# papuSpartan/stable-diffusion-webui-distributed

Measured on AMD Instinct MI355X. Metric: images/sec (whole node) SD1.5 txt2img 512x512 20-step batch=64 at 1/2/4/8 GPU, higher is better.
Workload: dtype bf16; 1 GPU; task=txt2img, model=sd15, global_batch=64, seq_len=512, resolution=512x512, denoise_steps=20, sampler=Euler a, parallelism=dp1 (benchmark-weighted batch shard)

## Files before the change

sdwd_amd/ops/hip/conv.hip:

```cpp
#include "common.h"
#include <map>
#include <mutex>
#include <tuple>

typedef __attribute__((ext_vector_type(4))) float f32x4c;

#define CONV_BM 128
#define CONV_BN 128
#define CONV_BK 64
#define TILE_ELEMS (CONV_BM * CONV_BK)


template <bool HAS_BIAS, bool HAS_RES, bool HAS_CB, int BN = 128,
          bool UPS = false, bool WRAP = false, bool FOLD = false>
__launch_bounds__(256, 2) __global__ void conv3x3_nhwc_bf16_kernel(
    const __hip_bfloat16 *__restrict__ X,
    const __hip_bfloat16 *__restrict__ Wt,
    const float *__restrict__ bias,
    const __hip_bfloat16 *__restrict__ Res,
    const __hip_bfloat16 *__restrict__ CB,
    const __hip_bfloat16 *__restrict__ Zero,
    __hip_bfloat16 *__restrict__ Y,
    int Nn, int H, int W, int Cin, int Cout, int Ho, int Wo, int stride,
    int ldY, float *__restrict__ GNP = nullptr, int wrap_h = 0,
    int wrap_w = 0) {
  __shared__ __align__(16) __bf16 smem[4 * TILE_ELEMS];

  static_assert(!(UPS && FOLD) && !(FOLD && (HAS_RES || HAS_CB)));
  const long M = FOLD ? (long)Nn * H * W : (long)Nn * Ho * Wo;
  constexpr int NJ = BN / 32;
  constexpr int BTILE = BN * CONV_BK;
  const int fa = FOLD ? (blockIdx.y >> 1) & 1 : 0;
  const int fb = FOLD ? blockIdx.y & 1 : 0;
  const long m0 =
      (((long)blockIdx.y + (long)blockIdx.z * 32768) >> (FOLD ? 2 : 0)) *
      CONV_BM;
  if constexpr (FOLD) {
    if (m0 >= M) return;
  }
  const int n0 = blockIdx.x * BN;

  const int tid = threadIdx.x;
  const int lane = tid % WAVE;
  const int wid = tid / WAVE;
  const int wm = (wid >> 1) * 64;
  const int wn = (wid & 1) * (BN / 2);

  long abase[4];
  int hs[4], ws[4];
  int bco[4];
  constexpr int NB = BN / 32;
  int nimg[4];
#pragma unroll
  for (int i = 0; i < 4; ++i) {
    const int row = i * 32 + wid * 8 + lane / 8;
    const long m = m0 + row;
    const long mm = (m < M) ? m : (M - 1);
    if constexpr (FOLD) {
      const unsigned q = (unsigned)mm / (unsigned)W;
      hs[i] = (int)(q % (unsigned)H) - 1 + fa;
      ws[i] = (int)((unsigned)mm - q * (unsigned)W) - 1 + fb;
      nimg[i] = 0;
      abase[i] = (mm + (long)(fa - 1) * W + (fb - 1)) * Cin;
    } else {
      const int n_img = (int)(mm / ((long)Ho * Wo));
      const int rem = (int)(mm % ((long)Ho * Wo));
      hs[i] = (rem / Wo) * stride;
      ws[i] = (rem % Wo) * stride;
      nimg[i] = n_img;
      abase[i] = (((long)n_img * H + hs[i]) * W + ws[i]) * Cin;
    }
    bco[i] = n0 + row;
  }
  const int schunk = lane % 8;

  const int kc_per_plane = Cin / CONV_BK;
  const int NT = (FOLD ? 4 : 9) * kc_per_plane;
  const int row_elems = W * Cin, img_elems = H * row_elems;
  (void)row_elems;
  (void)img_elems;

  auto stage = [&](int t, int b) {
    const int plane = t / kc_per_plane;
    const int kc = t % kc_per_plane;
    const int dy = FOLD ? plane >> 1 : plane / 3 - 1;
    const int dx = FOLD ? plane & 1 : plane % 3 - 1;
    const long poff = ((long)dy * W + dx) * Cin + (long)kc * CONV_BK;
    __bf16 *abuf = smem + b * (TILE_ELEMS + BTILE);
    __bf16 *bbuf = abuf + TILE_ELEMS;
#pragma unroll
    for (int i = 0; i < 4; ++i) {
      const int row = i * 32 + wid * 8 + lane / 8;
      const int sc = cswz(row, schunk);
      bool av;
      const __hip_bfloat16 *asrc;
      if constexpr (WRAP && UPS) {
        int vh = hs[i] + dy, vw = ws[i] + dx;
        if (wrap_h) {
          vh += vh < 0 ? 2 * H : 0;
          vh -= vh >= 2 * H ? 2 * H : 0;
        }
        if (wrap_w) {
          vw += vw < 0 ? 2 * W : 0;
          vw -= vw >= 2 * W ? 2 * W : 0;
        }
        av = vh >= 0 && vh < 2 * H && vw >= 0 && vw < 2 * W;
        asrc = av ? (X +
                     (((long)nimg[i] * H + (vh >> 1)) * W + (vw >> 1)) *
                         Cin +
                     (long)kc * CONV_BK + sc * 8)
                  : Zero;
      } else if constexpr (WRAP) {
        const int hh = hs[i] + dy, ww = ws[i] + dx;
        int dlt = 0;
        if (wrap_h) dlt += hh < 0 ? img_elems : (hh >= H ? -img_elems : 0);
        if (wrap_w) dlt += ww < 0 ? row_elems : (ww >= W ? -row_elems : 0);
        av = (wrap_h || (hh >= 0 && hh < H)) &&
             (wrap_w || (ww >= 0 && ww < W));
        asrc = av ? (X + abase[i] + poff + dlt + sc * 8) : Zero;
      } else if constexpr (UPS) {
        const int vh = hs[i] + dy, vw = ws[i] + dx;
        av = vh >= 0 && vh < 2 * H && vw >= 0 && vw < 2 * W;
        asrc = av ? (X +
                     (((long)nimg[i] * H + (vh >> 1)) * W + (vw >> 1)) *
                         Cin +
                     (long)kc * CONV_BK + sc * 8)
                  : Zero;
      } else {
        av = (hs[i] + dy >= 0) && (hs[i] + dy < H) &&
             (ws[i] + dx >= 0) && (ws[i] + dx < W);
        asrc = av ? (X + abase[i] + poff + sc * 8) : Zero;
      }
      (void)poff;
      __builtin_amdgcn_global_load_lds(
          (const __attribute__((address_space(1))) unsigned int *)asrc,
          (__attribute__((address_space(3))) unsigned int
               *)(abuf + i * 2048 + wid * 512),
          16, 0, 0);
      if (i < NB) {
        const bool bv = bco[i] < Cout;
        const __hip_bfloat16 *bsrc;
        if constexpr (FOLD) {
          bsrc = bv ? (Wt +
                       (((long)(2 * fa + fb) * Cout + bco[i]) * 4 + plane) *
                           Cin +
                       kc * CONV_BK + sc * 8)
                    : Zero;
        } else {
          bsrc = bv ? (Wt + (long)bco[i] * 9 * Cin + plane * Cin +
                       kc * CONV_BK + sc * 8)
                    : Zero;
        }
        __builtin_amdgcn_global_load_lds(
            (const __attribute__((address_space(1))) unsigned int *)bsrc,
            (__attribute__((address_space(3))) unsigned int
                 *)(bbuf + i * 2048 + wid * 512),
            16, 0, 0);
      }
    }
  };

  f32x4c acc[4][NJ];
#pragma unroll
  for (int i = 0; i < 4; ++i)
#pragma unroll
    for (int j = 0; j < NJ; ++j) acc[i][j] = (f32x4c){};

  stage(0, 0);
  if (NT > 1) stage(1, 1);

  const int l16 = lane % 16;
  const int kq = (lane / 16) * 8;

  for (int t = 0; t < NT; ++t) {
    if (t + 1 < NT)
      asm volatile("s_waitcnt vmcnt(%0)" :: "i"(4 + NB) : "memory");
    else
      asm volatile("s_waitcnt vmcnt(0)" ::: "memory");
    __builtin_amdgcn_s_barrier();

    const __bf16 *abuf = smem + (t & 1) * (TILE_ELEMS + BTILE);
    const __bf16 *bbuf = abuf + TILE_ELEMS;
#pragma unroll
    for (int s = 0; s < 2; ++s) {
      bf16x8 af[4], bf[NJ];
#pragma unroll
      for (int i = 0; i < 4; ++i) {
        const int am = wm + i * 16 + l16;
        const int ck = cswz(am, (s * 32 + kq) / 8);
        af[i] = *(const bf16x8 *)((const char *)(abuf + am * CONV_BK) +
                                  ck * 16);
      }
#pragma unroll
      for (int j = 0; j < NJ; ++j) {
        const int bn = wn + j * 16 + l16;
        const int ck = cswz(bn, (s * 32 + kq) / 8);
        bf[j] = *(const bf16x8 *)((const char *)(bbuf + bn * CONV_BK) +
                                  ck * 16);
      }
      __builtin_amdgcn_s_setprio(1);
#pragma unroll
      for (int i = 0; i < 4; ++i)
#pragma unroll
        for (int j = 0; j < NJ; ++j)
          acc[i][j] = __builtin_amdgcn_mfma_f32_16x16x32_bf16(
              af[i], bf[j], acc[i][j], 0, 0, 0);
      __builtin_amdgcn_s_setprio(0);
    }
    __builtin_amdgcn_s_barrier();
    if (t + 2 < NT) stage(t + 2, t & 1);
  }

  const int r4 = (lane / 16) * 4;
  float gs[NJ], gq[NJ];
#pragma unroll
  for (int j = 0; j < NJ; ++j) gs[j] = gq[j] = 0.0f;
#pragma unroll
  for (int i = 0; i < 4; ++i) {
#pragma unroll
    for (int j = 0; j < NJ; ++j) {
      const int co = n0 + wn + j * 16 + l16;
      if (co >= Cout) continue;
      const float bv = HAS_BIAS ? bias[co] : 0.0f;
#pragma unroll
      for (int r = 0; r < 4; ++r) {
        long m = m0 + wm + i * 16 + r4 + r;
        if (m >= M) continue;
        if constexpr (FOLD) {
          const unsigned q = (unsigned)m / (unsigned)W;
          const unsigned jw = (unsigned)m - q * (unsigned)W;
          m = (long)(2 * q + fa) * Wo + 2 * jw + fb;
        }
        float v = acc[i][j][r] + bv;
        if (HAS_CB) {
          const int ni = (int)(m / ((long)Ho * Wo));
          v += (float)CB[(long)ni * ldY + co];
        }
        if (HAS_RES) v += (float)Res[m * ldY + co];
        const __hip_bfloat16 vb = f2bf(v);
        Y[m * ldY + co] = vb;
        if (GNP) {
          const float vr = bf2f(vb);
          gs[j] += vr;
          gq[j] += vr * vr;
        }
      }
    }
  }
  if (GNP) {
    float *lds = (float *)smem;
#pragma unroll
    for (int j = 0; j < NJ; ++j) {
#pragma unroll
      for (int off = 16; off < 64; off <<= 1) {
        gs[j] += __shfl_down(gs[j], off, WAVE);
        gq[j] += __shfl_down(gq[j], off, WAVE);
      }
      if (lane < 16) {
        float *slot = lds + ((wid * NJ + j) * 16 + lane) * 2;
        slot[0] = gs[j];
        slot[1] = gq[j];
      }
    }
    __syncthreads();
    long gslot = (long)blockIdx.y + (long)blockIdx.z * 32768;
    if constexpr (FOLD) {
      const long tps = ((long)H * W) / CONV_BM, tp = gslot >> 2;
      gslot = ((tp / tps) * 4 + (gslot & 3)) * tps + tp % tps;
    }
    for (int c = tid; c < BN; c += 256) {
      const int co = n0 + c;
      if (co >= Cout) continue;
      const int h = c / (BN / 2);
      const int jj = (c % (BN / 2)) / 16;
      const int lc = c % 16;
      const float *s0 = lds + ((h * NJ + jj) * 16 + lc) * 2;
      const float *s1 = lds + (((h + 2) * NJ + jj) * 16 + lc) * 2;
      float *dst = GNP + (gslot * 2) * (long)ldY;
      dst[co] = s0[0] + s1[0];
      dst[ldY + co] = s0[1] + s1[1];
    }
  }
}

#ifdef __HIP_PLATFORM_AMD__
bool conv3x3_supported(long cin) { return cin % 64 == 0 && cin >= 64; }

std::tuple<long, long, bool> conv3x3_plan(long N, long H, long W, long Cin,
                                          long Cout, long stride,
                                          long force) {
  const long Ho = (H + 2 - 3) / stride + 1;
  const long Wo = (W + 2 - 3) / stride + 1;
  const long M = N * Ho * Wo;
  const long mtiles = (M + CONV_BM - 1) / CONV_BM;
  const long mt4 = (M + V4_BM - 1) / V4_BM;
  const bool v4_shape =
      force == 4 ? (Cin % 64 == 0 && Cout >= 256)
                 : (Cin <= 960 && Cout <= 640 && Cout >= 256 &&
                    mt4 * (Cout / 256) >= 256);
  const long nfull = (force == 2 || !v4_shape) ? 0 : Cout / 256;
  const long rem = Cout - nfull * 256;
  const bool bn64 =
      rem > 0 && (rem <= 64 || mtiles * ((rem + 127) / 128) < 512);
  return {nfull, rem, bn64};
}

static const __hip_bfloat16 *zero_page_for(const torch::Tensor &x) {
  static std::mutex mu;
  static std::map<int, torch::Tensor> pages;
  std::lock_guard<std::mutex> lock(mu);
  auto &page = pages[x.get_device()];
  if (!page.defined()) page = torch::zeros({64}, x.options());
  return (const __hip_bfloat16 *)page.data_ptr();
}

template <class F>
static void dispatch_bools(F &&f) {
  f();
}
template <class F, class... Rest>
static void dispatch_bools(F &&f, bool b, Rest... rest) {
  if (b)
    dispatch_bools([&](auto... cs) { f(std::true_type{}, cs...); }, rest...);
  else
    dispatch_bools([&](auto... cs) { f(std::false_type{}, cs...); }, rest...);
}

static dim3 conv_grid(long col_tiles, long mtiles) {
  return dim3((unsigned)col_tiles, (unsigned)std::min<long>(mtiles, 32768),
              (unsigned)((mtiles + 32767) / 32768));
}

struct ConvArgs {
  int N, Cin, H, W, Cout, Ho, Wo;
  long M;
  torch::Tensor y, gnp, bias_f32, cb_bf16;
  const __hip_bfloat16 *x, *w, *res = nullptr, *cb = nullptr, *zero;
  const float *bias = nullptr;
  __hip_bfloat16 *yp;
  float *gnp_ptr = nullptr;

  ConvArgs(const torch::Tensor &xt, const torch::Tensor &w_prep,
           const c10::optional<torch::Tensor> &bias_t,
           const c10::optional<torch::Tensor> &residual,
           const c10::optional<torch::Tensor> &chan_bias, int Ho_, int Wo_,
           bool collect_gn)
      : N(xt.size(0)), Cin(xt.size(1)), H(xt.size(2)), W(xt.size(3)),
        Cout(w_prep.size(0)), Ho(Ho_), Wo(Wo_), M((long)N * Ho_ * Wo_) {
    TORCH_CHECK(xt.is_contiguous(torch::MemoryFormat::ChannelsLast),
                "conv3x3: x must be channels_last");
    TORCH_CHECK(xt.scalar_type() == torch::kBFloat16);
    TORCH_CHECK(conv3x3_supported(Cin), "conv3x3: Cin % 64 != 0");
    y = torch::empty({N, Cout, Ho, Wo},
                     xt.options().memory_format(
                         torch::MemoryFormat::ChannelsLast));
    x = (const __hip_bfloat16 *)xt.data_ptr();
    w = (const __hip_bfloat16 *)w_prep.data_ptr();
    yp = (__hip_bfloat16 *)y.data_ptr();
    zero = zero_page_for(xt);
    if (bias_t.has_value()) {
      bias_f32 = bias_t->to(torch::kFloat).contiguous();
      bias = bias_f32.data_ptr<float>();
    }
    if (residual.has_value()) {
      TORCH_CHECK(
          residual->is_contiguous(torch::MemoryFormat::ChannelsLast));
      res = (const __hip_bfloat16 *)residual->data_ptr();
    }
    if (chan_bias.has_value()) {
      cb_bf16 = chan_bias->to(torch::kBFloat16).contiguous();
      cb = (const __hip_bfloat16 *)cb_bf16.data_ptr();
    }
    if (collect_gn && ((long)Ho * Wo) % 128 == 0) {
      gnp = torch::empty({M / 128, 2, (long)Cout},
                         xt.options().dtype(torch::kFloat));
      gnp_ptr = gnp.data_ptr<float>();
    }
  }

  std::tuple<torch::Tensor, c10::optional<torch::Tensor>> result() const {
    if (gnp.defined()) return {y, gnp};
    return {y, c10::nullopt};
  }
};

std::tuple<torch::Tensor, c10::optional<torch::Tensor>> conv3x3_nhwc(
    torch::Tensor x, torch::Tensor w_prep, c10::optional<torch::Tensor> bias,
    c10::optional<torch::Tensor> residual,
    c10::optional<torch::Tensor> chan_bias, long stride, bool collect_gn,
    long force, bool wrap_h = false, bool wrap_w = false) {
  const int Ho = (x.size(2) + 2 - 3) / stride + 1;
  const int Wo = (x.size(3) + 2 - 3) / stride + 1;
  ConvArgs a(x, w_prep, bias, residual, chan_bias, Ho, Wo, collect_gn);
  auto stream = cur_stream();
  const bool wrap = wrap_h || wrap_w;
  TORCH_CHECK(!wrap || (long)a.H * a.W * a.Cin < (1L << 31),
              "conv3x3: wrapped image too large");
  const auto [nfull, rem, bn64] =
      conv3x3_plan(a.N, a.H, a.W, a.Cin, a.Cout, stride, force);
  if (nfull > 0) {
    const int cols = (int)(nfull * 256);
    dispatch_bools(
        [&, cols](auto B, auto R, auto C, auto WR) {
          hipLaunchKernelGGL(
              (conv3x3_v4_kernel<decltype(B)::value, decltype(R)::value,
                                 decltype(C)::value, decltype(WR)::value>),
              conv_grid(cols / 256, (a.M + V4_BM - 1) / V4_BM), dim3(512), 0,
              stream, a.x, a.w, a.bias, a.res, a.cb, a.zero, a.yp, a.N, a.H,
              a.W, a.Cin, cols, a.Cout, a.Ho, a.Wo, (int)stride, a.gnp_ptr,
              (int)wrap_h, (int)wrap_w);
        },
        a.bias != nullptr, a.res != nullptr, a.cb != nullptr, wrap);
  }
  if (rem > 0) {
    const long co0 = nfull * 256;
    const int cols = (int)rem;
    dispatch_bools(
        [&, co0, cols](auto B, auto R, auto C, auto N64, auto WR) {
          constexpr int BN = decltype(N64)::value ? 64 : 128;
          hipLaunchKernelGGL(
              (conv3x3_nhwc_bf16_kernel<decltype(B)::value,
                                        decltype(R)::value,
                                        decltype(C)::value, BN, false,
                                        decltype(WR)::value>),
              conv_grid((cols + BN - 1) / BN,
                        (a.M + CONV_BM - 1) / CONV_BM),
              dim3(256), 0, stream, a.x, a.w + co0 * 9 * a.Cin,
              a.bias ? a.bias + co0 : nullptr, a.res ? a.res + co0 : nullptr,
              a.cb ? a.cb + co0 : nullptr, a.zero, a.yp + co0, a.N, a.H, a.W,
              a.Cin, cols, a.Ho, a.Wo, (int)stride, a.Cout,
              a.gnp_ptr ? a.gnp_ptr + co0 : nullptr, (int)wrap_h,
              (int)wrap_w);
        },
        a.bias != nullptr, a.res != nullptr, a.cb != nullptr, bn64, wrap);
  }
  return a.result();
}

static torch::Tensor launch_gn_tile_stats(const torch::Tensor &a,
                                          const torch::Tensor *b,
                                          torch::Tensor *out);

std::tuple<torch::Tensor, c10::optional<torch::Tensor>> ups2x_conv3x3(
    torch::Tensor x, torch::Tensor w_prep, c10::optional<torch::Tensor> bias,
    bool collect_gn, bool wrap_h = false, bool wrap_w = false,
    c10::optional<torch::Tensor> w_fold = c10::nullopt, bool fold = true) {
  auto stream = cur_stream();
  if (fold) {
    TORCH_CHECK(w_fold.has_value(),
                "ups2x_conv3x3: fold needs w_fold (fold_ups2x_weight)");
    const long H = x.size(2), W = x.size(3), Cin = x.size(1);
    const long Cout = w_prep.size(0), Mp = x.size(0) * H * W;
    TORCH_CHECK(w_fold->is_cuda() && w_fold->is_contiguous() &&
                    w_fold->scalar_type() == torch::kBFloat16 &&
                    w_fold->dim() == 5 && w_fold->size(0) == 4 &&
                    w_fold->size(1) == Cout && w_fold->size(2) == 2 &&
                    w_fold->size(3) == 2 && w_fold->size(4) == Cin,
                "ups2x_conv3x3: w_fold must be bf16 [4,Cout,2,2,Cin]");
    TORCH_CHECK(Mp < (1L << 31), "ups2x_conv3x3: too many source pixels");
    TORCH_CHECK(!(wrap_h || wrap_w) || H * W * Cin < (1L << 31),
                "ups2x_conv3x3: wrapped image too large");
    const bool epi_gn = collect_gn && (H * W) % CONV_BM == 0;
    ConvArgs a(x, w_prep, bias, c10::nullopt, c10::nullopt, 2 * H, 2 * W,
               epi_gn);
    const __hip_bfloat16 *wf = (const __hip_bfloat16 *)w_fold->data_ptr();
    dispatch_bools(
        [&](auto B, auto WR) {
          hipLaunchKernelGGL(
              (conv3x3_nhwc_bf16_kernel<decltype(B)::value, false, false,
                                        128, false, decltype(WR)::value,
                                        true>),
              conv_grid((a.Cout + CONV_BN - 1) / CONV_BN,
                        4 * ((Mp + CONV_BM - 1) / CONV_BM)),
              dim3(256), 0, stream, a.x, wf, a.bias, a.res, a.cb, a.zero,
              a.yp, a.N, a.H, a.W, a.Cin, a.Cout, a.Ho, a.Wo, 1, a.Cout,
              a.gnp_ptr, (int)wrap_h, (int)wrap_w);
        },
        a.bias != nullptr, wrap_h || wrap_w);
    if (collect_gn && !epi_gn && ((long)a.Ho * a.Wo) % 128 == 0 &&
        a.Cout % 8 == 0)
      a.gnp = launch_gn_tile_stats(a.y, nullptr, nullptr);
    return a.result();
  }
  ConvArgs a(x, w_prep, bias, c10::nullopt, c10::nullopt, 2 * x.size(2),
             2 * x.size(3), collect_gn);
  dispatch_bools(
      [&](auto B, auto WR) {
        hipLaunchKernelGGL(
            (conv3x3_nhwc_bf16_kernel<decltype(B)::value, false, false, 128,
                                      true, decltype(WR)::value>),
            conv_grid((a.Cout + CONV_BN - 1) / CONV_BN,
                      (a.M + CONV_BM - 1) / CONV_BM),
            dim3(256), 0, stream, a.x, a.w, a.bias, a.res, a.cb, a.zero,
            a.yp, a.N, a.H, a.W, a.Cin, a.Cout, a.Ho, a.Wo, 1, a.Cout,
            a.gnp_ptr, (int)wrap_h, (int)wrap_w);
      },
      a.bias != nullptr, wrap_h || wrap_w);
  return a.result();
}
#endif
```

sdwd_amd/ops/hip/conv_v4.hip:

```cpp
#include "common.h"

__device__ __forceinline__ int cswz(int row, int chunk) {
  return chunk ^ ((row >> 1) & 7);
}

#define V4_BM 256
#define V4_BN 256
#define V4_BK 64
#define V4_ATILE (V4_BM * V4_BK)

template <bool HAS_BIAS, bool HAS_RES, bool HAS_CB, bool WRAP = false>
__launch_bounds__(512, 2) __global__ void conv3x3_v4_kernel(
    const __hip_bfloat16 *__restrict__ X,
    const __hip_bfloat16 *__restrict__ Wt,
    const float *__restrict__ bias,
    const __hip_bfloat16 *__restrict__ Res,
    const __hip_bfloat16 *__restrict__ CB,
    const __hip_bfloat16 *__restrict__ Zero,
    __hip_bfloat16 *__restrict__ Y,
    int Nn, int H, int W, int Cin, int Cols, int ldY, int Ho, int Wo,
    int stride, float *__restrict__ GNP = nullptr, int wrap_h = 0,
    int wrap_w = 0) {
  __shared__ __align__(16) __bf16 smem[4 * V4_ATILE];

  const long M = (long)Nn * Ho * Wo;
  const long m0 =
      ((long)blockIdx.y + (long)blockIdx.z * 32768) * V4_BM;
  const int n0 = blockIdx.x * V4_BN;

  const int tid = threadIdx.x;
  const int lane = tid % WAVE;
  const int wid = tid / WAVE;
  const int wm = (wid >> 2) * 128;
  const int wn = (wid & 3) * 64;

  const int prow = tid / 8;
  const int schunk = tid % 8;
  long abase[4];
  int hs[4], ws[4];
  int bco[4];
#pragma unroll
  for (int i = 0; i < 4; ++i) {
    const long m = m0 + prow + 64 * i;
    const long mm = (m < M) ? m : (M - 1);
    const int n_img = (int)(mm / ((long)Ho * Wo));
    const int rem = (int)(mm % ((long)Ho * Wo));
    hs[i] = (rem / Wo) * stride;
    ws[i] = (rem % Wo) * stride;
    abase[i] = (((long)n_img * H + hs[i]) * W + ws[i]) * Cin;
    bco[i] = n0 + prow + 64 * i;
  }

  const int kc_per_plane = Cin / V4_BK;
  const int NT = 9 * kc_per_plane;
  const int row_elems = W * Cin, img_elems = H * row_elems;
  (void)row_elems;
  (void)img_elems;

  auto stage8 = [&](int t, int b) {
    const int plane = t / kc_per_plane;
    const int kc = t % kc_per_plane;
    const int dy = plane / 3 - 1, dx = plane % 3 - 1;
    const long poff = ((long)dy * W + dx) * Cin + (long)kc * V4_BK;
    __bf16 *abuf = smem + b * (2 * V4_ATILE);
    __bf16 *bbuf = abuf + V4_ATILE;
    const int sc = schunk;
    constexpr int PIECES[8] = {4, 5, 6, 7, 0, 1, 2, 3};
#pragma unroll
    for (int k = 0; k < 8; ++k) {
      const int i = PIECES[k];
      if (i < 4) {
        const int row = prow + 64 * i;
        const int swz = cswz(row, sc);
        bool av;
        const __hip_bfloat16 *asrc;
        if constexpr (WRAP) {
          const int hh = hs[i] + dy, ww = ws[i] + dx;
          int dlt = 0;
          if (wrap_h) dlt += hh < 0 ? img_elems : (hh >= H ? -img_elems : 0);
          if (wrap_w) dlt += ww < 0 ? row_elems : (ww >= W ? -row_elems : 0);
          av = (wrap_h || (hh >= 0 && hh < H)) &&
               (wrap_w || (ww >= 0 && ww < W));
          asrc = av ? (X + abase[i] + poff + dlt + swz * 8) : Zero;
        } else {
          av = (hs[i] + dy >= 0) && (hs[i] + dy < H) &&
               (ws[i] + dx >= 0) && (ws[i] + dx < W);
          asrc = av ? (X + abase[i] + poff + swz * 8) : Zero;
        }
        __builtin_amdgcn_global_load_lds(
            (const __attribute__((address_space(1))) unsigned int *)asrc,
            (__attribute__((address_space(3))) unsigned int
                 *)(abuf + (long)i * 4096 + (long)tid * 8),
            16, 0, 0);
      } else {
        const int bi = i - 4;
        const int row = prow + 64 * bi;
        const int swz = cswz(row, sc);
        const bool bv = bco[bi] < Cols;
        const __hip_bfloat16 *bsrc =
            bv ? (Wt + (long)bco[bi] * 9 * Cin + plane * Cin +
                  kc * V4_BK + swz * 8)
               : Zero;
        __builtin_amdgcn_global_load_lds(
            (const __attribute__((address_space(1))) unsigned int *)bsrc,
            (__attribute__((address_space(3))) unsigned int
                 *)(bbuf + (long)bi * 4096 + (long)tid * 8),
            16, 0, 0);
      }
    }
  };

  f32x4 acc[8][4];
#pragma unroll
  for (int i = 0; i < 8; ++i)
#pragma unroll
    for (int j = 0; j < 4; ++j) acc[i][j] = (f32x4){};

  stage8(0, 0);
  asm volatile("s_waitcnt vmcnt(0)" ::: "memory");
  __builtin_amdgcn_s_barrier();

  const int l16 = lane % 16;
  const int kq4 = lane / 16;

  for (int t = 0; t < NT; ++t) {
    const __bf16 *abuf = smem + (t & 1) * (2 * V4_ATILE);
    const __bf16 *bbuf = abuf + V4_ATILE;
#pragma unroll
    for (int ph = 0; ph < 4; ++ph) {
      const int mh = ph >> 1, nh = ph & 1;
      bf16x8 af[4][2], bf[2][2];
#pragma unroll
      for (int s = 0; s < 2; ++s) {
#pragma unroll
        for (int i = 0; i < 4; ++i) {
          const int ar = wm + mh * 64 + i * 16 + l16;
          const int ck = cswz(ar, s * 4 + kq4);
          af[i][s] = *(const bf16x8 *)((const char *)(abuf +
                                                      (long)ar * V4_BK) +
                                       ck * 16);
        }
#pragma unroll
        for (int j = 0; j < 2; ++j) {
          const int br = wn + nh * 32 + j * 16 + l16;
          const int ck = cswz(br, s * 4 + kq4);
          bf[j][s] = *(const bf16x8 *)((const char *)(bbuf +
                                                      (long)br * V4_BK) +
                                       ck * 16);
        }
      }
      if (ph == 0 && t + 1 < NT) stage8(t + 1, (t + 1) & 1);
      __builtin_amdgcn_s_barrier();
      __builtin_amdgcn_s_setprio(1);
#pragma unroll
      for (int s = 0; s < 2; ++s)
#pragma unroll
        for (int i = 0; i < 4; ++i)
#pragma unroll
          for (int j = 0; j < 2; ++j)
            acc[mh * 4 + i][nh * 2 + j] =
                __builtin_amdgcn_mfma_f32_16x16x32_bf16(
                    af[i][s], bf[j][s], acc[mh * 4 + i][nh * 2 + j], 0, 0,
                    0);
      __builtin_amdgcn_s_setprio(0);
      if (ph == 3 && t + 1 < NT)
        asm volatile("s_waitcnt vmcnt(0)" ::: "memory");
      __builtin_amdgcn_s_barrier();
    }
  }

  const int r4 = (lane / 16) * 4;
  float gs[4], gq[4];
#pragma unroll
  for (int j = 0; j < 4; ++j) gs[j] = gq[j] = 0.0f;
#pragma unroll
  for (int i = 0; i < 8; ++i) {
#pragma unroll
    for (int j = 0; j < 4; ++j) {
      const int co = n0 + wn + (j >> 1) * 32 + (j & 1) * 16 + l16;
      if (co >= Cols) continue;
      const float bv = HAS_BIAS ? bias[co] : 0.0f;
#pragma unroll
      for (int r = 0; r < 4; ++r) {
        const long m = m0 + wm + (i >> 2) * 64 + (i & 3) * 16 + r4 + r;
        if (m >= M) continue;
        float v = acc[i][j][r] + bv;
        if (HAS_CB) {
          const int ni = (int)(m / ((long)Ho * Wo));
          v += (float)CB[(long)ni * ldY + co];
        }
        if (HAS_RES) v += (float)Res[m * ldY + co];
        const __hip_bfloat16 vb = f2bf(v);
        Y[m * ldY + co] = vb;
        if (GNP) {
          const float vr = bf2f(vb);
          gs[j] += vr;
          gq[j] += vr * vr;
        }
      }
    }
  }
  if (GNP) {
    float *lds = (float *)smem;
#pragma unroll
    for (int j = 0; j < 4; ++j) {
#pragma unroll
      for (int off = 16; off < 64; off <<= 1) {
        gs[j] += __shfl_down(gs[j], off, WAVE);
        gq[j] += __shfl_down(gq[j], off, WAVE);
      }
      if (lane < 16) {
        float *slot = lds + ((wid * 4 + j) * 16 + lane) * 2;
        slot[0] = gs[j];
        slot[1] = gq[j];
      }
    }
    __syncthreads();
    const long mt128 = m0 / 128;
    for (int c = tid; c < V4_BN; c += 512) {
      const int co = n0 + c;
      if (co >= Cols) continue;
      const int q = c / 64;
      const int o = c % 64;
      const int jj = (o / 32) * 2 + (o % 32) / 16;
      const int lc = c % 16;
      const float *s0 = lds + ((q * 4 + jj) * 16 + lc) * 2;
      const float *s1 = lds + (((q + 4) * 4 + jj) * 16 + lc) * 2;
      float *d0 = GNP + (mt128 * 2) * (long)ldY;
      d0[co] = s0[0];
      d0[ldY + co] = s0[1];
      if ((mt128 + 1) * 128 < M) {
        float *d1 = GNP + ((mt128 + 1) * 2) * (long)ldY;
        d1[co] = s1[0];
        d1[ldY + co] = s1[1];
      }
    }
  }
}
```

Before: 17.25 images/sec.

## Stage conv epilogue through LDS for vectorized 16-byte output stores

Adds a shared epilogue helper that, for full tiles, writes bias/residual/channel-bias-adjusted bf16 results into per-wave LDS strips and then stores them to global memory as 16-byte vectors instead of scattered 2-byte stores. Residual and channel-bias loads are prefetched one row-group ahead, and the channel-bias division is dropped when a tile lies within a single image. Bias can now be passed as bf16 or fp32 without a host-side conversion. The partial-tile path keeps the scalar epilogue, and the GroupNorm scratch area moves in LDS to avoid overlapping the strips.

New measurement: 18.14 images/sec, median of 6. +5.1%, better.

```diff
diff --git a/sdwd_amd/ops/hip/conv.hip b/sdwd_amd/ops/hip/conv.hip
--- a/sdwd_amd/ops/hip/conv.hip
+++ b/sdwd_amd/ops/hip/conv.hip
@@ -1,4 +1,5 @@
 #include "common.h"
+#include "conv_epilogue.h"
 #include <map>
 #include <mutex>
 #include <tuple>
@@ -16,13 +17,13 @@
 __launch_bounds__(256, 2) __global__ void conv3x3_nhwc_bf16_kernel(
     const __hip_bfloat16 *__restrict__ X,
     const __hip_bfloat16 *__restrict__ Wt,
-    const float *__restrict__ bias,
+    const void *__restrict__ bias,
     const __hip_bfloat16 *__restrict__ Res,
     const __hip_bfloat16 *__restrict__ CB,
     const __hip_bfloat16 *__restrict__ Zero,
     __hip_bfloat16 *__restrict__ Y,
     int Nn, int H, int W, int Cin, int Cout, int Ho, int Wo, int stride,
-    int ldY, float *__restrict__ GNP = nullptr, int wrap_h = 0,
+    int ldY, int flags, float *__restrict__ GNP = nullptr, int wrap_h = 0,
     int wrap_w = 0) {
   __shared__ __align__(16) __bf16 smem[4 * TILE_ELEMS];
 
@@ -215,40 +216,81 @@
   float gs[NJ], gq[NJ];
 #pragma unroll
   for (int j = 0; j < NJ; ++j) gs[j] = gq[j] = 0.0f;
-#pragma unroll
-  for (int i = 0; i < 4; ++i) {
+  const bool full =
+      (flags & CONV_F_VEC) && m0 + CONV_BM <= M && n0 + BN <= Cout;
+  if (full) {
+    const int uw = __builtin_amdgcn_readfirstlane(wid);
+    const int uwm = (uw >> 1) * 64, uwn = (uw & 1) * (BN / 2);
+    float bv[NJ], cbv[NJ];
 #pragma unroll
     for (int j = 0; j < NJ; ++j) {
-      const int co = n0 + wn + j * 16 + l16;
-      if (co >= Cout) continue;
-      const float bv = HAS_BIAS ? bias[co] : 0.0f;
-#pragma unroll
-      for (int r = 0; r < 4; ++r) {
-        long m = m0 + wm + i * 16 + r4 + r;
-        if (m >= M) continue;
-        if constexpr (FOLD) {
-          const unsigned q = (unsigned)m / (unsigned)W;
-          const unsigned jw = (unsigned)m - q * (unsigned)W;
-          m = (long)(2 * q + fa) * Wo + 2 * jw + fb;
+      bv[j] = HAS_BIAS ? conv_bias_at(bias, flags, n0 + uwn + j * 16 + l16)
+                       : 0.0f;
+      cbv[j] = 0.0f;
+    }
+    const unsigned HoWo = (unsigned)(Ho * Wo);
+    bool cb_one = true;
+    unsigned rem0 = 0;
+    const __hip_bfloat16 *cbw = nullptr;
+    if constexpr (HAS_CB) {
+      const long ni0 = m0 / (long)HoWo;
+      const unsigned remb = (unsigned)(m0 - ni0 * (long)HoWo);
+      cb_one = remb + CONV_BM <= HoWo;
+      rem0 = remb + uwm;
+      cbw = CB + ni0 * (long)ldY + n0 + uwn;
+#pragma unroll
+      for (int j = 0; j < NJ; ++j) cbv[j] = (float)cbw[j * 16 + l16];
+    }
+    const long mw = m0 + uwm;
+    const __hip_bfloat16 *resw =
+        HAS_RES ? Res + mw * (long)ldY + n0 + uwn : nullptr;
+    __hip_bfloat16 *yw =
+        FOLD ? Y + n0 + uwn : Y + mw * (long)ldY + n0 + uwn;
+    char *wl = (char *)smem + wid * conv_epi_bytes<NJ>;
+    if (cb_one)
+      conv_epi_strip<HAS_RES, HAS_CB, true, FOLD, NJ, false>(
+          acc, bv, cbv, cbw, rem0, HoWo, resw, yw, mw, W, Wo, fa, fb,
+          (unsigned)ldY, wl, lane, gs, gq);
+    else
+      conv_epi_strip<HAS_RES, HAS_CB, false, FOLD, NJ, false>(
+          acc, bv, cbv, cbw, rem0, HoWo, resw, yw, mw, W, Wo, fa, fb,
+          (unsigned)ldY, wl, lane, gs, gq);
+  } else {
+#pragma unroll
+    for (int i = 0; i < 4; ++i) {
+#pragma unroll
+      for (int j = 0; j < NJ; ++j) {
+        const int co = n0 + wn + j * 16 + l16;
+        if (co >= Cout) continue;
+        const float bv = HAS_BIAS ? conv_bias_at(bias, flags, co) : 0.0f;
+#pragma unroll
+        for (int r = 0; r < 4; ++r) {
+          long m = m0 + wm + i * 16 + r4 + r;
+          if (m >= M) continue;
+          if constexpr (FOLD) {
+            const unsigned q = (unsigned)m / (unsigned)W;
+            const unsigned jw = (unsigned)m - q * (unsigned)W;
+            m = (long)(2 * q + fa) * Wo + 2 * jw + fb;
+          }
+          float v = acc[i][j][r] + bv;
+          if (HAS_CB) {
+            const int ni = (int)(m / ((long)Ho * Wo));
+            v += (float)CB[(long)ni * ldY + co];
+          }
+          if (HAS_RES) v += (float)Res[m * ldY + co];
+          const __hip_bfloat16 vb = f2bf(v);
+          Y[m * ldY + co] = vb;
+          if (GNP) {
+            const float vr = bf2f(vb);
+            gs[j] += vr;
+            gq[j] += vr * vr;
+          }
         }
-        float v = acc[i][j][r] + bv;
-        if (HAS_CB) {
-          const int ni = (int)(m / ((long)Ho * Wo));
-          v += (float)CB[(long)ni * ldY + co];
-        }
-        if (HAS_RES) v += (float)Res[m * ldY + co];
-        const __hip_bfloat16 vb = f2bf(v);
-        Y[m * ldY + co] = vb;
-        if (GNP) {
-          const float vr = bf2f(vb);
-          gs[j] += vr;
-          gq[j] += vr * vr;
-        }
       }
     }
   }
   if (GNP) {
-    float *lds = (float *)smem;
+    float *lds = (float *)((char *)smem + 4 * conv_epi_bytes<4>);
 #pragma unroll
     for (int j = 0; j < NJ; ++j) {
 #pragma unroll
@@ -336,9 +378,19 @@
   long M;
   torch::Tensor y, gnp, bias_f32, cb_bf16;
   const __hip_bfloat16 *x, *w, *res = nullptr, *cb = nullptr, *zero;
-  const float *bias = nullptr;
+  const char *bias = nullptr;
+  int bias_esize = 4;
   __hip_bfloat16 *yp;
   float *gnp_ptr = nullptr;
+
+  const void *bias_at(long co0) const {
+    return bias ? bias + co0 * bias_esize : nullptr;
+  }
+  int flags(long co0, long cols) const {
+    const bool vec = cols % 8 == 0 && Cout % 8 == 0 &&
+                     (reinterpret_cast<uintptr_t>(yp + co0) & 15) == 0;
+    return (vec ? CONV_F_VEC : 0) | (bias_esize == 2 ? CONV_F_BIAS_BF16 : 0);
+  }
 
   ConvArgs(const torch::Tensor &xt, const torch::Tensor &w_prep,
            const c10::optional<torch::Tensor> &bias_t,
@@ -358,9 +410,19 @@
     w = (const __hip_bfloat16 *)w_prep.data_ptr();
     yp = (__hip_bfloat16 *)y.data_ptr();
     zero = zero_page_for(xt);
+    TORCH_CHECK(Cout < (1 << 20), "conv3x3: too many output channels");
+    TORCH_CHECK((long)Ho * Wo < (1L << 30), "conv3x3: output image too large");
     if (bias_t.has_value()) {
-      bias_f32 = bias_t->to(torch::kFloat).contiguous();
-      bias = bias_f32.data_ptr<float>();
+      TORCH_CHECK(bias_t->numel() == Cout, "conv3x3: bias must be [Cout]");
+      const auto bt = bias_t->scalar_type();
+      if ((bt == torch::kBFloat16 || bt == torch::kFloat) &&
+          bias_t->is_contiguous()) {
+        bias_f32 = *bias_t;
+        bias_esize = bt == torch::kBFloat16 ? 2 : 4;
+      } else {
+        bias_f32 = bias_t->to(torch::kFloat).contiguous();
+      }
+      bias = (const char *)bias_f32.data_ptr();
     }
     if (residual.has_value()) {
       TORCH_CHECK(
@@ -406,9 +468,9 @@
               (conv3x3_v4_kernel<decltype(B)::value, decltype(R)::value,
                                  decltype(C)::value, decltype(WR)::value>),
               conv_grid(cols / 256, (a.M + V4_BM - 1) / V4_BM), dim3(512), 0,
-              stream, a.x, a.w, a.bias, a.res, a.cb, a.zero, a.yp, a.N, a.H,
-              a.W, a.Cin, cols, a.Cout, a.Ho, a.Wo, (int)stride, a.gnp_ptr,
-              (int)wrap_h, (int)wrap_w);
+              stream, a.x, a.w, a.bias_at(0), a.res, a.cb, a.zero, a.yp, a.N,
+              a.H, a.W, a.Cin, cols, a.Cout, a.Ho, a.Wo, (int)stride,
+              a.flags(0, cols), a.gnp_ptr, (int)wrap_h, (int)wrap_w);
         },
         a.bias != nullptr, a.res != nullptr, a.cb != nullptr, wrap);
   }
@@ -426,11 +488,11 @@
               conv_grid((cols + BN - 1) / BN,
                         (a.M + CONV_BM - 1) / CONV_BM),
               dim3(256), 0, stream, a.x, a.w + co0 * 9 * a.Cin,
-              a.bias ? a.bias + co0 : nullptr, a.res ? a.res + co0 : nullptr,
+              a.bias_at(co0), a.res ? a.res + co0 : nullptr,
               a.cb ? a.cb + co0 : nullptr, a.zero, a.yp + co0, a.N, a.H, a.W,
               a.Cin, cols, a.Ho, a.Wo, (int)stride, a.Cout,
-              a.gnp_ptr ? a.gnp_ptr + co0 : nullptr, (int)wrap_h,
-              (int)wrap_w);
+              a.flags(co0, cols), a.gnp_ptr ? a.gnp_ptr + co0 : nullptr,
+              (int)wrap_h, (int)wrap_w);
         },
         a.bias != nullptr, a.res != nullptr, a.cb != nullptr, bn64, wrap);
   }
@@ -472,9 +534,10 @@
                                         true>),
               conv_grid((a.Cout + CONV_BN - 1) / CONV_BN,
                         4 * ((Mp + CONV_BM - 1) / CONV_BM)),
-              dim3(256), 0, stream, a.x, wf, a.bias, a.res, a.cb, a.zero,
-              a.yp, a.N, a.H, a.W, a.Cin, a.Cout, a.Ho, a.Wo, 1, a.Cout,
-              a.gnp_ptr, (int)wrap_h, (int)wrap_w);
+              dim3(256), 0, stream, a.x, wf, a.bias_at(0), a.res, a.cb,
+              a.zero, a.yp, a.N, a.H, a.W, a.Cin, a.Cout, a.Ho, a.Wo, 1,
+              a.Cout, a.flags(0, a.Cout), a.gnp_ptr, (int)wrap_h,
+              (int)wrap_w);
         },
         a.bias != nullptr, wrap_h || wrap_w);
     if (collect_gn && !epi_gn && ((long)a.Ho * a.Wo) % 128 == 0 &&
@@ -491,9 +554,9 @@
                                       true, decltype(WR)::value>),
             conv_grid((a.Cout + CONV_BN - 1) / CONV_BN,
                       (a.M + CONV_BM - 1) / CONV_BM),
-            dim3(256), 0, stream, a.x, a.w, a.bias, a.res, a.cb, a.zero,
-            a.yp, a.N, a.H, a.W, a.Cin, a.Cout, a.Ho, a.Wo, 1, a.Cout,
-            a.gnp_ptr, (int)wrap_h, (int)wrap_w);
+            dim3(256), 0, stream, a.x, a.w, a.bias_at(0), a.res, a.cb,
+            a.zero, a.yp, a.N, a.H, a.W, a.Cin, a.Cout, a.Ho, a.Wo, 1,
+            a.Cout, a.flags(0, a.Cout), a.gnp_ptr, (int)wrap_h, (int)wrap_w);
       },
       a.bias != nullptr, wrap_h || wrap_w);
   return a.result();
diff --git a/sdwd_amd/ops/hip/conv_epilogue.h b/sdwd_amd/ops/hip/conv_epilogue.h
--- /dev/null
+++ b/sdwd_amd/ops/hip/conv_epilogue.h
@@ -0,0 +1,103 @@
+#pragma once
+#include "common.h"
+
+#define CONV_F_VEC 1
+#define CONV_F_BIAS_BF16 2
+
+__device__ __forceinline__ float conv_bias_at(const void *bias, int flags,
+                                              int co) {
+  return (flags & CONV_F_BIAS_BF16)
+             ? bf2f(((const __hip_bfloat16 *)bias)[co])
+             : ((const float *)bias)[co];
+}
+
+template <int NJ>
+constexpr int conv_epi_stride = NJ * 32 + 16;
+template <int NJ>
+constexpr int conv_epi_bytes = 64 * conv_epi_stride<NJ>;
+
+template <bool HAS_RES, bool HAS_CB, bool CB_ONE, bool FOLD, int NJ,
+          bool TIGHT>
+__device__ __forceinline__ void conv_epi_strip(
+    const f32x4 (&acc)[4][NJ], const float (&bv)[NJ], const float (&cbv)[NJ],
+    const __hip_bfloat16 *__restrict__ cbw, unsigned rem0, unsigned HoWo,
+    const __hip_bfloat16 *__restrict__ resw, __hip_bfloat16 *__restrict__ yw,
+    long mrow, int W, int Wo, int fa, int fb, unsigned ldY, char *wl,
+    int lane, float (&gs)[NJ], float (&gq)[NJ]) {
+  constexpr int STRIDE = conv_epi_stride<NJ>;
+  constexpr bool LOADS = HAS_RES || (HAS_CB && !CB_ONE);
+  constexpr bool AHEAD = !(TIGHT && HAS_CB && !CB_ONE);
+  const unsigned l16 = lane % 16, r4 = (lane / 16) * 4;
+  float rv[2][NJ][4], cv[2][NJ][4];
+  unsigned voff[4];
+#pragma unroll
+  for (int r = 0; r < 4; ++r) voff[r] = ((r4 + r) * ldY + l16) * 2;
+  auto fetch = [&](int i, int b) {
+    const char *ri = (const char *)resw + (size_t)(i * 16) * ldY * 2;
+#pragma unroll
+    for (int r = 0; r < 4; ++r) {
+      unsigned coff = l16 * 2;
+      if constexpr (HAS_CB && !CB_ONE)
+        coff += ((rem0 + i * 16 + r4 + r) / HoWo) * ldY * 2;
+#pragma unroll
+      for (int j = 0; j < NJ; ++j) {
+        if constexpr (HAS_RES)
+          rv[b][j][r] =
+              (float)*(const __hip_bfloat16 *)((ri + voff[r]) + j * 32);
+        if constexpr (HAS_CB)
+          cv[b][j][r] = CB_ONE ? cbv[j]
+                               : (float)*(const __hip_bfloat16 *)(
+                                     ((const char *)cbw + coff) + j * 32);
+      }
+    }
+  };
+  if constexpr (AHEAD) fetch(0, 0);
+#pragma unroll
+  for (int i = 0; i < 4; ++i) {
+    if constexpr (AHEAD) {
+      if (i + 1 < 4) fetch(i + 1, (i + 1) & 1);
+    } else {
+      fetch(i, i & 1);
+    }
+    if constexpr (TIGHT && LOADS) __builtin_amdgcn_sched_barrier(0);
+#pragma unroll
+    for (int j = 0; j < NJ; ++j) {
+#pragma unroll
+      for (int r = 0; r < 4; ++r) {
+        float v = acc[i][j][r] + bv[j];
+        if constexpr (HAS_CB) v += cv[i & 1][j][r];
+        if constexpr (HAS_RES) v += rv[i & 1][j][r];
+        const __hip_bfloat16 vb = f2bf(v);
+        *(__hip_bfloat16 *)(wl + (i * 16 + r4 + r) * STRIDE +
+                            (j * 16 + l16) * 2) = vb;
+        const float vr = bf2f(vb);
+        gs[j] += vr;
+        gq[j] += vr * vr;
+      }
+    }
+    if constexpr (TIGHT && LOADS) __builtin_amdgcn_sched_barrier(0);
+  }
+  asm volatile("s_waitcnt lgkmcnt(0)" ::: "memory");
+  constexpr int CH = NJ * 2;
+  constexpr int RP = 64 / CH;
+  const unsigned prow = lane / CH, pch = lane % CH;
+  uint4 ov[CH];
+#pragma unroll
+  for (int p = 0; p < CH; ++p)
+    ov[p] = *(const uint4 *)(wl + (p * RP + prow) * STRIDE + pch * 16);
+  const unsigned soff = (prow * ldY + pch * 8) * 2;
+#pragma unroll
+  for (int p = 0; p < CH; ++p) {
+    const unsigned row = p * RP + prow;
+    if constexpr (FOLD) {
+      const unsigned m = (unsigned)mrow + row;
+      const unsigned q = m / (unsigned)W;
+      const unsigned jw = m - q * (unsigned)W;
+      const long orow = (long)(2 * q + fa) * Wo + 2 * jw + fb;
+      *(uint4 *)(yw + orow * (long)ldY + pch * 8) = ov[p];
+    } else {
+      *(uint4 *)(((char *)yw + (size_t)(p * RP) * ldY * 2) + soff) = ov[p];
+    }
+  }
+  asm volatile("s_waitcnt lgkmcnt(0)" ::: "memory");
+}
diff --git a/sdwd_amd/ops/hip/conv_v4.hip b/sdwd_amd/ops/hip/conv_v4.hip
--- a/sdwd_amd/ops/hip/conv_v4.hip
+++ b/sdwd_amd/ops/hip/conv_v4.hip
@@ -1,4 +1,5 @@
 #include "common.h"
+#include "conv_epilogue.h"
 
 __device__ __forceinline__ int cswz(int row, int chunk) {
   return chunk ^ ((row >> 1) & 7);
@@ -13,13 +14,13 @@
 __launch_bounds__(512, 2) __global__ void conv3x3_v4_kernel(
     const __hip_bfloat16 *__restrict__ X,
     const __hip_bfloat16 *__restrict__ Wt,
-    const float *__restrict__ bias,
+    const void *__restrict__ bias,
     const __hip_bfloat16 *__restrict__ Res,
     const __hip_bfloat16 *__restrict__ CB,
     const __hip_bfloat16 *__restrict__ Zero,
     __hip_bfloat16 *__restrict__ Y,
     int Nn, int H, int W, int Cin, int Cols, int ldY, int Ho, int Wo,
-    int stride, float *__restrict__ GNP = nullptr, int wrap_h = 0,
+    int stride, int flags, float *__restrict__ GNP = nullptr, int wrap_h = 0,
     int wrap_w = 0) {
   __shared__ __align__(16) __bf16 smem[4 * V4_ATILE];
 
@@ -173,35 +174,80 @@
   float gs[4], gq[4];
 #pragma unroll
   for (int j = 0; j < 4; ++j) gs[j] = gq[j] = 0.0f;
-#pragma unroll
-  for (int i = 0; i < 8; ++i) {
+  const bool full =
+      (flags & CONV_F_VEC) && m0 + V4_BM <= M && n0 + V4_BN <= Cols;
+  if (full) {
+    const int uw = __builtin_amdgcn_readfirstlane(wid);
+    const int uwm = (uw >> 2) * 128, uwn = (uw & 3) * 64;
+    float bv[4], cbv[4];
 #pragma unroll
     for (int j = 0; j < 4; ++j) {
-      const int co = n0 + wn + (j >> 1) * 32 + (j & 1) * 16 + l16;
-      if (co >= Cols) continue;
-      const float bv = HAS_BIAS ? bias[co] : 0.0f;
-#pragma unroll
-      for (int r = 0; r < 4; ++r) {
-        const long m = m0 + wm + (i >> 2) * 64 + (i & 3) * 16 + r4 + r;
-        if (m >= M) continue;
-        float v = acc[i][j][r] + bv;
-        if (HAS_CB) {
-          const int ni = (int)(m / ((long)Ho * Wo));
-          v += (float)CB[(long)ni * ldY + co];
-        }
-        if (HAS_RES) v += (float)Res[m * ldY + co];
-        const __hip_bfloat16 vb = f2bf(v);
-        Y[m * ldY + co] = vb;
-        if (GNP) {
-          const float vr = bf2f(vb);
-          gs[j] += vr;
-          gq[j] += vr * vr;
+      bv[j] = HAS_BIAS ? conv_bias_at(bias, flags, n0 + uwn + j * 16 + l16)
+                       : 0.0f;
+      cbv[j] = 0.0f;
+    }
+    const unsigned HoWo = (unsigned)(Ho * Wo);
+    bool cb_one = true;
+    unsigned remb = 0;
+    const __hip_bfloat16 *cbw = nullptr;
+    if constexpr (HAS_CB) {
+      const long ni0 = m0 / (long)HoWo;
+      remb = (unsigned)(m0 - ni0 * (long)HoWo);
+      cb_one = remb + V4_BM <= HoWo;
+      cbw = CB + ni0 * (long)ldY + n0 + uwn;
+#pragma unroll
+      for (int j = 0; j < 4; ++j) cbv[j] = (float)cbw[j * 16 + l16];
+    }
+    char *wl = (char *)smem + wid * conv_epi_bytes<4>;
+#pragma unroll
+    for (int s = 0; s < 2; ++s) {
+      const long mw = m0 + uwm + s * 64;
+      const f32x4(&sa)[4][4] = *reinterpret_cast<const f32x4(*)[4][4]>(
+          &acc[s * 4]);
+      const __hip_bfloat16 *resw =
+          HAS_RES ? Res + mw * (long)ldY + n0 + uwn : nullptr;
+      __hip_bfloat16 *yw = Y + mw * (long)ldY + n0 + uwn;
+      const unsigned rem0 = remb + uwm + s * 64;
+      if (cb_one)
+        conv_epi_strip<HAS_RES, HAS_CB, true, false, 4, true>(
+            sa, bv, cbv, cbw, rem0, HoWo, resw, yw, mw, 0, 0, 0, 0,
+            (unsigned)ldY, wl, lane, gs, gq);
+      else
+        conv_epi_strip<HAS_RES, HAS_CB, false, false, 4, true>(
+            sa, bv, cbv, cbw, rem0, HoWo, resw, yw, mw, 0, 0, 0, 0,
+            (unsigned)ldY, wl, lane, gs, gq);
+    }
+  } else {
+#pragma unroll
+    for (int i = 0; i < 8; ++i) {
+#pragma unroll
+      for (int j = 0; j < 4; ++j) {
+        const int co = n0 + wn + (j >> 1) * 32 + (j & 1) * 16 + l16;
+        if (co >= Cols) continue;
+        const float bv = HAS_BIAS ? conv_bias_at(bias, flags, co) : 0.0f;
+#pragma unroll
+        for (int r = 0; r < 4; ++r) {
+          const long m = m0 + wm + (i >> 2) * 64 + (i & 3) * 16 + r4 + r;
+          if (m >= M) continue;
+          float v = acc[i][j][r] + bv;
+          if (HAS_CB) {
+            const int ni = (int)(m / ((long)Ho * Wo));
+            v += (float)CB[(long)ni * ldY + co];
+          }
+          if (HAS_RES) v += (float)Res[m * ldY + co];
+          const __hip_bfloat16 vb = f2bf(v);
+          Y[m * ldY + co] = vb;
+          if (GNP) {
+            const float vr = bf2f(vb);
+            gs[j] += vr;
+            gq[j] += vr * vr;
+          }
         }
       }
     }
   }
   if (GNP) {
-    float *lds = (float *)smem;
+    float *lds = (float *)((char *)smem + 8 * conv_epi_bytes<4>);
 #pragma unroll
     for (int j = 0; j < 4; ++j) {
 #pragma unroll
```
